# jdidion/atropos

Measured on AMD Instinct MI355X. Metric: reads/s (whole node) 150 bp SE adapter-align, higher is better.
Workload: dtype int32

## Files before the change

### atropos_amd/csrc/piece_kernels.hip

```cpp
#include "locate_fast.hpp"
#include "piece_filter.hpp"
#include "jit.hpp"

namespace atr {

void launch_fast_scan(FastWork wk, hipStream_t st);
int launch_fast_dp(const atr_aligner *a, const uint4 *packed, const int32_t *lens, long long nreads, int nchunks,
                   int max_len, uint4 *out, FastWork wk, const LinkedArgs *la, int idx, int count, hipStream_t st, bool planes, bool one_stream);

template <int NW, bool RAGGED, int WW>
__global__ __launch_bounds__(256) __attribute__((amdgpu_waves_per_eu(ATR_PIECE_WAVES(NW), 8))) void piece_filter_kernel(
    const LocateParams p, const FilterParams fp, const PieceParams pp, const uint4 *__restrict__ planes,
    const int32_t *__restrict__ lens, long long nreads, int max_len, uint4 *__restrict__ out, FastWork wk) {
    piece_filter_body<NW, RAGGED, WW>(p, fp, pp, planes, lens, nreads, max_len, out, wk);
}

__global__ __launch_bounds__(256) void piece_scatter_kernel(long long nreads, int m, FastWork wk) {
    __shared__ uint32_t s_cur[FILTER_BINS + 1], s_tmp[256];
    const long long ntiles = (nreads + 63) >> 6;
    long long t0, t1;
    block_tiles(ntiles, t0, t1, wk.nused);
    const uint2 *list = wk.tmp + t0 * 64;
    const uint32_t count = wk.lcount[blockIdx.x];
    const uint32_t mine = threadIdx.x < FILTER_BINS ? wk.counts[(size_t)blockIdx.x * FILTER_BINS + threadIdx.x] : 0u;
    const uint2 first = threadIdx.x < count ? list[threadIdx.x] : make_uint2(0u, 0u);
    if (wk.fused) {
        fused_bin_bases(wk, s_cur, s_tmp);
        if (threadIdx.x < FILTER_BINS) s_cur[threadIdx.x] += mine;
    } else if (threadIdx.x < FILTER_BINS) s_cur[threadIdx.x] = fast_slot0(wk, threadIdx.x);
    __syncthreads();
    for (uint32_t i = threadIdx.x; i < count; i += 256) {
        const uint2 e = i == threadIdx.x ? first : list[i];
        const uint32_t slot = atomicAdd(&s_cur[window_bin(e.y & ~PIECE_NODENSE, m, true)], 1u);
        wk.order[slot] = e;
        wk.dref[slot] = (uint32_t)(t0 * 64) + i;
    }
}

template <int NW, bool RAGGED, int WW>
static int piece_resident_blocks() {
    static thread_local int cached_dev = -1, cached = 0;
    int dev = 0;
    if (hipGetDevice(&dev) != hipSuccess) return 1024;
    if (dev != cached_dev) {
        int per_cu = 0, cus = 0;
        if (hipOccupancyMaxActiveBlocksPerMultiprocessor(&per_cu, piece_filter_kernel<NW, RAGGED, WW>, 256, 0) != hipSuccess || per_cu < 1) per_cu = 2;
        if (hipDeviceGetAttribute(&cus, hipDeviceAttributeMultiprocessorCount, dev) != hipSuccess || cus < 1) cus = 256;
        cached = std::min(FAST_BLOCKS, per_cu * cus);
        cached_dev = dev;
    }
    return cached;
}

template <int NW, int WW>
static void launch_piece_filter_w(const atr_aligner *a, const FilterParams &fp, const PieceParams &pp, const uint4 *planes,
                                  const int32_t *lens, long long nreads, int max_len, uint4 *out, FastWork &wk, hipStream_t st) {
    const long long want = ((nreads + 63) / 64 + 3) / 4;
    if (lens) {
        wk.nused = (int)std::max<long long>(1, std::min<long long>(piece_resident_blocks<NW, true, WW>(), want));
        hipLaunchKernelGGL((piece_filter_kernel<NW, true, WW>), dim3(wk.nused), dim3(256), 0, st, a->p, fp, pp, planes, lens, nreads, max_len, out, wk);
    } else {
        wk.nused = (int)std::max<long long>(1, std::min<long long>(piece_resident_blocks<NW, false, WW>(), want));
        hipLaunchKernelGGL((piece_filter_kernel<NW, false, WW>), dim3(wk.nused), dim3(256), 0, st, a->p, fp, pp, planes, lens, nreads, max_len, out, wk);
    }
}
template <int NW>
static void launch_piece_filter(const atr_aligner *a, const FilterParams &fp, const PieceParams &pp, const uint4 *planes,
                                const int32_t *lens, long long nreads, int max_len, uint4 *out, FastWork &wk, hipStream_t st) {
    if (pp.window > PIECE_WINDOW || pp.nb > 5 || fp.rows > 32) launch_piece_filter_w<NW, 3>(a, fp, pp, planes, lens, nreads, max_len, out, wk, st);
    else launch_piece_filter_w<NW, 2>(a, fp, pp, planes, lens, nreads, max_len, out, wk, st);
}

int piece_ragged_len(int max_len) { return 32 * ((max_len + 31) / 32); }
bool piece_applies(const atr_aligner *a, int max_len, FilterParams *fp_out, PieceParams *pp_out) {
    if (!a->filterable || max_len < 1) return false;
    const FilterParams &fp = aligner_piece_filter_params(a);
    PieceParams pp;
    if (!piece_params(a->codes, a->p.m, fp.rows, a->p.k, a->flags, a->wildcard_ref || a->wildcard_query,
                      a->table_kind == ATR_TABLE_CUSTOM, fp.thr_row, max_len, pp, a->p.thr, a->p.min_overlap, fp.cert, a->p.indel)) return false;
    const int nw = (max_len + 31) / 32;
    if (nw < 3 || nw > 10) return false;
    if (fp_out) *fp_out = fp;
    if (pp_out) *pp_out = pp;
    return true;
}

static const jit::SpecKernel *piece_spec_for(const atr_aligner *a, const FilterParams &fp, const PieceParams &pp, bool ragged,
                                             int max_len, long long nreads, bool force, int ascii_stride = 0) {
    const int pol = jit::policy();
    if (pol == 0) return nullptr;
    const int nw = (max_len + 31) / 32;
    a->planes_seen += nreads;
    const bool compile = force || pol == 1 || a->planes_seen >= jit::min_reads();
    return jit::spec_kernel(a, fp, pp, nw, ragged, ragged ? 32 * nw : max_len, compile, ascii_stride);
}

static bool tail_spec_enabled() {
    const char *x = getenv("ATR_TAIL_SPEC");
    return !(x && x[0] == '0');
}

int prepare_locate_planes(const atr_aligner *a, int max_len, bool ragged) {
    FilterParams fp;
    PieceParams pp;
    if (!piece_applies(a, ragged ? piece_ragged_len(max_len) : max_len, &fp, &pp)) return 0;
    return piece_spec_for(a, fp, pp, ragged, max_len, 0, true) != nullptr ? 1 : 0;
}

int launch_planes_prepass(const atr_aligner *a, const uint4 *planes, const int32_t *lens, long long nreads, int max_len,
                          uint4 *out, void *work, hipStream_t st, int grid_div, PlanesCall *pc) {
    FilterParams fp;
    PieceParams pp;
    if (!piece_applies(a, lens ? piece_ragged_len(max_len) : max_len, &fp, &pp)) return (int)hipErrorInvalidValue;
    FastWork wk = fast_carve(work, nreads);
    wk.lpw = nreads <= 8192 ? 0 : 64;
    const int nw = (max_len + 31) / 32;
    const jit::SpecKernel *sk = piece_spec_for(a, fp, pp, lens != nullptr, max_len, nreads, false);
    wk.fused = fast_fused_scan() ? 1 : 0;
    if (wk.fused) {
        const hipError_t rc = hipMemsetAsync(wk.chunks, 0, (size_t)wk.nbins * 4, st);
        if (rc != hipSuccess) return (int)rc;
    }
    if (sk) {
        const long long want = ((nreads + 63) / 64 + 3) / 4;
        wk.nused = (int)std::max<long long>(1, std::min<long long>(std::max(1, sk->resident / std::max(1, grid_div)), want));
        const hipError_t rc = jit::spec_launch(sk, wk.nused, planes, lens, nreads, max_len, out, wk, st);
        if (rc != hipSuccess) return (int)rc;
    } else {
        switch (nw) {
        case 3: launch_piece_filter<3>(a, fp, pp, planes, lens, nreads, max_len, out, wk, st); break;
        case 4: launch_piece_filter<4>(a, fp, pp, planes, lens, nreads, max_len, out, wk, st); break;
        case 5: launch_piece_filter<5>(a, fp, pp, planes, lens, nreads, max_len, out, wk, st); break;
        case 6: launch_piece_filter<6>(a, fp, pp, planes, lens, nreads, max_len, out, wk, st); break;
        case 7: launch_piece_filter<7>(a, fp, pp, planes, lens, nreads, max_len, out, wk, st); break;
        case 8: launch_piece_filter<8>(a, fp, pp, planes, lens, nreads, max_len, out, wk, st); break;
        case 9: launch_piece_filter<9>(a, fp, pp, planes, lens, nreads, max_len, out, wk, st); break;
        default: launch_piece_filter<10>(a, fp, pp, planes, lens, nreads, max_len, out, wk, st); break;
        }
    }
    pc->wk = wk;
    pc->nw = nw;
    pc->tail = sk ? (void *)sk->tail : nullptr;
    return (int)hipGetLastError();
}

int launch_planes_tail(const atr_aligner *a, const uint4 *planes, const int32_t *lens, long long nreads, int max_len, uint4 *out,
                       const PlanesCall &pc, hipStream_t st, bool one_stream) {
    FastWork wk = pc.wk;
    if (!wk.fused) launch_fast_scan(wk, st);
    hipLaunchKernelGGL(piece_scatter_kernel, dim3(wk.nused), dim3(256), 0, st, nreads, a->p.m, wk);
    if (pc.tail && !one_stream && tail_spec_enabled()) {
        {
            const bool small = nreads <= 65536;
            const int win_blocks = (int)std::max<long long>(1, std::min<long long>((nreads + 3) / 4, 1024));
            const int band_blocks = (int)std::max<long long>(1, std::min<long long>(small ? (nreads + 3) / 4 : (nreads + 255) / 256, 4096));
            const hipError_t rc = jit::tail_launch((hipFunction_t)pc.tail, win_blocks, band_blocks, planes, lens, pc.nw, max_len, out, wk, st);
            return rc != hipSuccess ? (int)rc : (int)hipGetLastError();
        }
    }
    return launch_fast_dp(a, planes, lens, nreads, pc.nw, max_len, out, wk, nullptr, 0, 1, st, true, one_stream);
}

int launch_locate_planes_shared(const atr_aligner *a, const uint4 *planes, const int32_t *lens, long long nreads, int max_len,
                                uint4 *out, void *work, hipStream_t st, int grid_div, bool one_stream) {
    PlanesCall pc;
    const int rc = launch_planes_prepass(a, planes, lens, nreads, max_len, out, work, st, grid_div, &pc);
    if (rc != 0) return rc;
    return launch_planes_tail(a, planes, lens, nreads, max_len, out, pc, st, one_stream);
}

int launch_locate_ascii_fused(const atr_aligner *a, const uint8_t *ascii, long long row_stride, const int32_t *lens, long long nreads,
                              int max_len, const uint8_t table[256], uint4 *planes, uint4 *out, void *work, hipStream_t st) {
    FilterParams fp;
    PieceParams pp;
    if (!piece_applies(a, lens ? piece_ragged_len(max_len) : max_len, &fp, &pp)) return 1;
    const int nw = (max_len + 31) / 32;
    static const bool off = [] { const char *x = getenv("ATR_ASCII_FUSED"); return x && x[0] == '0'; }();
    if (off || nw > 8 || row_stride < max_len || row_stride > 256 || ((uintptr_t)ascii & 1)) return 1;
    const jit::SpecKernel *sk = piece_spec_for(a, fp, pp, lens != nullptr, max_len, nreads, jit::policy() != 0, (int)row_stride);
    if (!sk) return 1;
    FastWork wk = fast_carve(work, nreads);
    wk.lpw = nreads <= 8192 ? 0 : 64;
    wk.fused = fast_fused_scan() ? 1 : 0;
    if (wk.fused) {
        const hipError_t rc = hipMemsetAsync(wk.chunks, 0, (size_t)wk.nbins * 4, st);
        if (rc != hipSuccess) return (int)rc;
    }
    const long long want = ((nreads + 63) / 64 + 3) / 4;
    wk.nused = (int)std::max<long long>(1, std::min<long long>(sk->resident, want));
    const hipError_t rc = jit::spec_launch_ascii(sk, wk.nused, ascii, lens, nreads, max_len, out, wk, planes, table, st);
    if (rc != hipSuccess) return (int)rc;
    PlanesCall pc;
    pc.wk = wk;
    pc.nw = nw;
    pc.tail = (void *)sk->tail;
    return launch_planes_tail(a, planes, lens, nreads, max_len, out, pc, st, false);
}

int launch_locate_planes(const atr_aligner *a, const uint4 *planes, const int32_t *lens, long long nreads, int max_len, uint4 *out,
                         void *work, hipStream_t st) {
    return launch_locate_planes_shared(a, planes, lens, nreads, max_len, out, work, st, 1, false);
}

}
```

### atropos_amd/csrc/tail_filter.hpp

```cpp
#ifndef ATR_TAIL_FILTER_HPP
#define ATR_TAIL_FILTER_HPP

#ifdef ATR_HOST_EMU
#include "filter_core.hpp"
#else
#include "fast_work.hpp"
#endif

namespace atr {

#ifndef ATR_TAIL_ROWS_UNROLL
#define ATR_TAIL_ROWS_UNROLL 8
#endif
#ifndef ATR_TAIL_WINDOW_UNROLL
#define ATR_TAIL_WINDOW_UNROLL 2
#endif
constexpr int TAIL_ROWS_UNROLL = ATR_TAIL_ROWS_UNROLL;
static_assert(TAIL_ROWS_UNROLL >= 8 && TAIL_ROWS_UNROLL % 8 == 0, "the feed position is a compile-time place of the body");

template <bool AND_MODE, int ND>
ATR_DEV void tail_band_row(const Uniform &u, uint32_t rrep, uint32_t qw0, uint32_t qw1, uint32_t (&band)[BAND_W]) {
    const uint32_t inf = ((uint32_t)INIT_COST_CAP << CSH) | ORG_BIAS;
    uint32_t m0 = nibble_any(AND_MODE ? (qw0 & rrep) : (qw0 ^ rrep));
    uint32_t m1 = ND > 8 ? nibble_any(AND_MODE ? (qw1 & rrep) : (qw1 ^ rrep)) : 0u;
    if (AND_MODE) { m0 = ~m0; m1 = ~m1; }
    uint32_t left = inf;
#pragma unroll
    for (int c = 0; c < ND; ++c) {
        const uint32_t bit = atr_bfe1(c < 8 ? m0 : m1, 4 * (c & 7) + 3);
        const uint32_t cd = atr_mad24(bit, COST1 + MATCH1, band[c]);
        const uint32_t up = c + 1 < ND ? band[c + 1 < ND ? c + 1 : 0] : inf;
        const uint32_t nw = atr_minu(atr_minu(cd, left + u.delw), up + u.insw) & ~PRIO_MASK;
        band[c] = nw;
        left = nw;
    }
}

struct TailLast {
    int cap_lo, top, r0, at0, n, cindel;
    bool active;
};

template <bool AND_MODE, int ND, int ROWS_MAX, bool LAST>
ATR_DEV void tail_band_sweep(const Uniform &u, const uint32_t *rreps, int rows, const uint32_t *ns, int nss,
                             uint32_t (&band)[BAND_W], const TailLast &tl, const int16_t *thr, Best &best) {
    uint32_t qw0 = ns[0], qw1 = ns[(size_t)nss];
    uint32_t feed = ns[(size_t)2 * nss];
#pragma unroll 1
    for (int i0 = 0; i0 < ROWS_MAX; i0 += TAIL_ROWS_UNROLL) {
        if (i0 >= rows) break;
#pragma unroll
        for (int t = 0; t < TAIL_ROWS_UNROLL; ++t) {
            const int i = i0 + t + 1;
            if (i <= ROWS_MAX && i <= rows) {
                tail_band_row<AND_MODE, ND>(u, rreps[i - 1], qw0, qw1, band);
                if (LAST && i >= tl.cap_lo) {
                    const int at = tl.at0 - i;
                    if (tl.active && i <= tl.top && i >= tl.r0 && (u.er || i == u.m)) {
                        uint32_t cell = band[0];
#pragma unroll
                        for (int c = 1; c < ND; ++c) cell = at == c ? band[c] : cell;
                        if (cell < u.klimit) consider<true>(best, cell, i, tl.n, u.min_overlap, thr, tl.cindel);
                    }
                }
                qw0 = (qw0 >> 4) | (qw1 << 28);
                qw1 = (qw1 >> 4) | (feed << 28);
                feed >>= 4;
                if (((t + 1) & 7) == 0) {
                    const int k = 2 + (i >> 3);
                    feed = k < BAND_STREAM ? ns[(size_t)k * nss] : 0u;
                }
            }
        }
    }
}

ATR_DEV void tail_band_record(const Best &best, int none_cost, uint32_t rec[4]) {
    const int cost = (int)(best.word >> CSH);
    int refstart = 0, querystart = 0, refstop = -1, querystop = 0, matches = 0, errors = 0;
    if (cost != none_cost) {
        const int origin = (int)(best.word & ORG_MASK) - (int)ORG_BIAS;
        if (origin >= 0) querystart = origin; else refstart = -origin;
        refstop = best.ref_stop; querystop = best.query_stop;
        matches = best.matches; errors = cost;
    }
    rec[0] = (uint32_t)(refstart & 0xFFFF) | ((uint32_t)(refstop & 0xFFFF) << 16);
    rec[1] = (uint32_t)(querystart & 0xFFFF) | ((uint32_t)(querystop & 0xFFFF) << 16);
    rec[2] = (uint32_t)(matches & 0xFFFF) | ((uint32_t)(errors & 0xFFFF) << 16);
    rec[3] = 0;
}

template <bool AND_MODE, int ROWS_MAX>
ATR_DEV void tail_band_locate(const Uniform &u, const uint32_t *rreps, bool noindel, const uint32_t *ns, int nss, int n,
                              uint32_t ww, int smax, const int16_t *thr, uint32_t rec[4]) {
    const int dlo = window_lo(ww);
    uint32_t band[BAND_W];
#pragma unroll
    for (int c = 0; c < BAND_W; ++c) band[c] = ORG_BIAS + (uint32_t)(dlo + c);
    Best best;
    best.key = COST_FIELD_MAX - (u.m + n);
    best.word = (uint32_t)(u.m + n) << CSH;
    best.ref_stop = u.m; best.query_stop = n; best.matches = 0;
    const TailLast none = {0, 0, 0, 0, 0, 0, false};
    if (smax < 8) tail_band_sweep<AND_MODE, 8, ROWS_MAX, false>(u, rreps, u.m, ns, nss, band, none, thr, best);
    else if (smax < 10) tail_band_sweep<AND_MODE, 10, ROWS_MAX, false>(u, rreps, u.m, ns, nss, band, none, thr, best);
    else if (smax < 12) tail_band_sweep<AND_MODE, 12, ROWS_MAX, false>(u, rreps, u.m, ns, nss, band, none, thr, best);
    else if (smax < 14) tail_band_sweep<AND_MODE, 14, ROWS_MAX, false>(u, rreps, u.m, ns, nss, band, none, thr, best);
    else tail_band_sweep<AND_MODE, 16, ROWS_MAX, false>(u, rreps, u.m, ns, nss, band, none, thr, best);
    const int cindel = noindel ? 0 : u.indel;
#pragma unroll
    for (int c = 0; c < BAND_W; ++c) {
        const int j = dlo + u.m + c;
        if (c <= smax && band[c] < u.klimit && j <= n) consider<true>(best, band[c], u.m, j, u.min_overlap, thr, cindel);
    }
    tail_band_record(best, u.m + n, rec);
}

template <bool AND_MODE, int ROWS_MAX>
ATR_DEV void tail_band_locate_last(const Uniform &u, const uint32_t *rreps, bool noindel, const uint32_t *ns, int nss, int n,
                                   uint32_t ww, bool active, int smax, int rows_max, int cap_lo, const int16_t *thr,
                                   uint32_t rec[4]) {
    const int dlo = window_lo(ww), top = window_rows(ww), r0 = top - last_band_span(ww), at0 = n - dlo;
    uint32_t band[BAND_W];
#pragma unroll
    for (int c = 0; c < BAND_W; ++c) band[c] = ORG_BIAS + (uint32_t)(dlo + c);
    Best best, bm;
    best.key = COST_FIELD_MAX - (u.m + n);
    best.word = (uint32_t)(u.m + n) << CSH;
    best.ref_stop = u.m; best.query_stop = n; best.matches = 0;
    bm = best;
    const int cindel = noindel ? 0 : u.indel;
    const TailLast tl = {cap_lo, top, r0, at0, n, cindel, active};
    if (smax < 4) tail_band_sweep<AND_MODE, 4, ROWS_MAX, true>(u, rreps, rows_max, ns, nss, band, tl, thr, best);
    else if (smax < 6) tail_band_sweep<AND_MODE, 6, ROWS_MAX, true>(u, rreps, rows_max, ns, nss, band, tl, thr, best);
    else if (smax < 8) tail_band_sweep<AND_MODE, 8, ROWS_MAX, true>(u, rreps, rows_max, ns, nss, band, tl, thr, best);
    else if (smax < 10) tail_band_sweep<AND_MODE, 10, ROWS_MAX, true>(u, rreps, rows_max, ns, nss, band, tl, thr, best);
    else if (smax < 12) tail_band_sweep<AND_MODE, 12, ROWS_MAX, true>(u, rreps, rows_max, ns, nss, band, tl, thr, best);
    else if (smax < 14) tail_band_sweep<AND_MODE, 14, ROWS_MAX, true>(u, rreps, rows_max, ns, nss, band, tl, thr, best);
    else tail_band_sweep<AND_MODE, 16, ROWS_MAX, true>(u, rreps, rows_max, ns, nss, band, tl, thr, best);
    if (last_band_rowm(ww) && rows_max == u.m) {
        const int width = last_band_width(ww);
#pragma unroll
        for (int c = 0; c < BAND_W; ++c) {
            const int j = dlo + u.m + c;
            if (c <= width && band[c] < u.klimit && j <= n) consider<true>(bm, band[c], u.m, j, u.min_overlap, thr, cindel);
        }
        if (bm.key >= best.key) best = bm;
    }
    tail_band_record(best, u.m + n, rec);
}

#if defined(ATR_TAIL_SPEC) && !defined(ATR_HOST_EMU)
#include "tail_spec_config.h"

__device__ __forceinline__ Uniform tail_uniform() {
    Uniform u;
    u.m = tspec::M; u.k = tspec::K; u.p0 = tspec::MT - tspec::M; u.indel = tspec::INDEL; u.min_overlap = tspec::MIN_OVERLAP;
    u.sr = (tspec::FLAGS & ATR_START_WITHIN_SEQ1) != 0; u.sq = (tspec::FLAGS & ATR_START_WITHIN_SEQ2) != 0;
    u.er = (tspec::FLAGS & ATR_STOP_WITHIN_SEQ1) != 0;  u.eq = (tspec::FLAGS & ATR_STOP_WITHIN_SEQ2) != 0;
    u.first_p = u.p0 + (u.er ? 0 : u.m);
    u.insw = (uint32_t)u.indel * COST1 + PRIO_INS;
    u.delw = (uint32_t)u.indel * COST1 + PRIO_DEL;
    u.klimit = (uint32_t)(u.k + 1) << CSH;
    return u;
}

__device__ __forceinline__ int tail_lanes_per_wave(long long tasks, long long grid_waves, int fixed) {
    if (fixed) return fixed;
    int lpw = 1;
    while (lpw < 64 && (long long)lpw * grid_waves < tasks) lpw <<= 1;
    return lpw;
}

struct TailShared {
    int16_t thr[tspec::M + 2];
    uint32_t init[tspec::MT + 1];
    __attribute__((aligned(16))) uint32_t nm[16][4];
    uint32_t stream[4][BAND_STREAM][64];
    uint32_t spread[4][256];
};

__device__ __forceinline__ void tail_band_blocks(TailShared &S, int block, int nblocks, const uint4 *__restrict__ packed,
                                                 const int32_t *__restrict__ lens, int nchunks, int max_len,
                                                 uint4 *__restrict__ out, const FastWork &wk) {
    constexpr int M = tspec::M;
    const Uniform u = tail_uniform();
    const long long total = (long long)wk.binbase[BAND_BINS];
    const int lane = threadIdx.x & 63, wave = __builtin_amdgcn_readfirstlane((int)(threadIdx.x >> 6));
    const long long stride = (long long)nblocks * 4;
    const int lpw = tail_lanes_per_wave(total, stride, wk.lpw);
    const long long nwaves = (total + lpw - 1) / lpw;
    uint32_t *ns = &S.stream[wave][0][lane];
    long long wv = (long long)block * 4 + wave;
    if (wv >= nwaves) return;
    auto slot_of = [&](long long w) { return w * lpw + lane; };
    auto live_of = [&](long long w) { return w < nwaves && lane < lpw && slot_of(w) < total; };
    auto dense_of = [&](long long w, uint2 task) { return live_of(w) && (task.y & PIECE_NODENSE) == 0u; };
    const uint4 zero4 = make_uint4(0u, 0u, 0u, 0u);
    uint2 task = live_of(wv) ? wk.order[slot_of(wv)] : make_uint2(0u, 0u);
    uint32_t di = live_of(wv) ? wk.dref[slot_of(wv)] : 0u;
    uint2 task1 = live_of(wv + stride) ? wk.order[slot_of(wv + stride)] : make_uint2(0u, 0u);
    uint32_t di1 = live_of(wv + stride) ? wk.dref[slot_of(wv + stride)] : 0u;
    uint4 a = dense_of(wv, task) ? wk.tdata[2 * (size_t)di] : zero4, b = dense_of(wv, task) ? wk.tdata[2 * (size_t)di + 1] : zero4;
    int n = live_of(wv) ? (lens ? lens[task.x] : max_len) : 0;
    for (; wv < nwaves; wv += stride) {
        const bool live = live_of(wv);
        const long long r = (long long)task.x;
        const uint32_t ww = task.y;
        const bool dense1 = dense_of(wv + stride, task1);
        const uint4 a1 = dense1 ? wk.tdata[2 * (size_t)di1] : zero4, b1 = dense1 ? wk.tdata[2 * (size_t)di1 + 1] : zero4;
        const int n1 = live_of(wv + stride) ? (lens ? lens[task1.x] : max_len) : 0;
        const bool live2 = live_of(wv + 2 * stride);
        const uint2 task2 = live2 ? wk.order[slot_of(wv + 2 * stride)] : make_uint2(0u, 0u);
        const uint32_t di2 = live2 ? wk.dref[slot_of(wv + 2 * stride)] : 0u;

        const bool last = live && window_scan(ww);
        const bool any_last = wave_max_i32(last ? 1 : 0) != 0, any_rowm = wave_max_i32(live && !last ? 1 : 0) != 0;
        const int s_lane = (live && !last) ? window_hi(ww) - u.m + u.k - window_lo(ww) : 0;
        const int smax = min(BAND_W - 1, wave_max_i32(s_lane));
        const bool dense = live && (ww & PIECE_NODENSE) == 0u;
        if (dense) {
            ns[0] = a.x; ns[64] = a.y; ns[128] = a.z; ns[192] = a.w;
            ns[256] = b.x; ns[320] = b.y; ns[384] = b.z; ns[448] = b.w;
        }
        if (wave_max_i32(live && !dense ? 1 : 0) != 0) {
            const uint32_t *q = (const uint32_t *)(packed + ((size_t)(r >> 6) * nchunks) * 64 + (r & 63));
            if (live && !dense) band_stage_planes(q, nchunks, window_lo(ww), ns, 64, S.spread, band_stream_dwords(M));
        }
        uint32_t rec[4] = {0xFFFF0000u, 0u, 0u, 0u};
        if (any_rowm) tail_band_locate<tspec::AND_MODE, M>(u, tspec::RREP, tspec::NOINDEL, ns, 64, n, ww, smax, S.thr, rec);
        if (any_last) {
            const int smax_l = min(BAND_W - 1, wave_max_i32(last ? last_band_width(ww) : 0));
            const int rows_max = wave_max_i32(last ? (last_band_rowm(ww) ? u.m : window_rows(ww)) : 0);
            const int cap_lo = wave_min_i32(last ? window_rows(ww) - last_band_span(ww) : 0x7fffffff);
            uint32_t rec_l[4];
            tail_band_locate_last<tspec::AND_MODE, M>(u, tspec::RREP, tspec::NOINDEL, ns, 64, n, ww, last, smax_l, min(rows_max, M), cap_lo, S.thr, rec_l);
            if (last) { rec[0] = rec_l[0]; rec[1] = rec_l[1]; rec[2] = rec_l[2]; rec[3] = rec_l[3]; }
        }
        if (live) out[r] = make_uint4(rec[0], rec[1], rec[2], rec[3]);
        task = task1; di = di1; a = a1; b = b1; n = n1;
        task1 = task2; di1 = di2;
    }
}

template <int W>
__device__ __forceinline__ void tail_load_mask(uint32_t (&nm)[W], const uint32_t (*s_nm)[4], uint32_t q) {
#pragma unroll
    for (int w = 0; w < W; ++w) nm[w] = s_nm[q][w];
}

__device__ __forceinline__ void tail_window_blocks(TailShared &S, int block, int nblocks, const uint4 *__restrict__ packed,
                                                   const int32_t *__restrict__ lens, int nchunks, int max_len,
                                                   uint4 *__restrict__ out, const FastWork &wk) {
    constexpr int MT = tspec::MT;
    constexpr bool NOINDEL = tspec::NOINDEL;
    const Uniform u = tail_uniform();
    const int16_t *s_thr = S.thr;
    const uint32_t *s_init = S.init;
    const uint32_t (*s_nm)[4] = S.nm;
    const uint32_t (*s_spread)[256] = S.spread;
    const long long first = (long long)wk.binbase[BAND_BINS], total = (long long)wk.binbase[FILTER_BINS];
    if (total <= first) return;
    const int lane = threadIdx.x & 63;
    const int lpw = tail_lanes_per_wave(total - first, (long long)nblocks * 4, wk.lpw);
    const long long nwaves = (total - first + lpw - 1) / lpw;
    __builtin_amdgcn_s_setprio(3);
    for (long long wv = (long long)block * 4 + __builtin_amdgcn_readfirstlane((int)(threadIdx.x >> 6)); wv < nwaves;
         wv += (long long)nblocks * 4) {
        const long long slot = first + wv * lpw + lane;
        const bool live = lane < lpw && slot < total;
        const uint2 task = live ? wk.order[slot] : make_uint2(0u, 0u);
        const long long r = (long long)task.x;
        const uint32_t ww = task.y;
        const int n = live ? (lens ? lens[r] : max_len) : 0;
        const int j_lo = window_lo(ww), j_hi = live ? window_hi(ww) : 0;
        const bool has_window = live && j_hi > j_lo;
        const int jlo = wave_min_i32(live ? j_lo : 0x7fffffff);
        const int jhi = wave_max_i32(has_window ? j_hi : 0);
        const int rows_w = wave_max_i32(live ? window_rows(ww) : 0);
        const int plimit = u.p0 + rows_w;
        const bool head = !(u.sr && jlo == 0);
        const bool rows_wave = __builtin_amdgcn_readfirstlane((int)(first + wv * lpw >= (long long)wk.binbase[ROWS_BIN0])) != 0;
        const bool tri = rows_wave && head && lens == nullptr;

        LaneState<MT> L;
        const uint4 *tp = packed + ((size_t)(r >> 6) * nchunks) * 64 + (r & 63);

        if (lens != nullptr && rows_wave && !u.sr) {
            const int shift = live ? max_len - n : 0;
            const int v0 = wave_min_i32(live ? j_lo + shift : 0x7fffffff);
            if (max_len - v0 <= TAIL_COLUMNS && v0 < max_len) {
                const int s_top_t = wave_max_i32(shift);
                lane_init_window<MT, NOINDEL>(L, u, max_len, v0, live ? max_len : 0, live && window_scan(ww), s_init, s_thr);
                uint32_t tb[TAIL_COLUMNS / 8];
                {
                    const int dlo = n - TAIL_COLUMNS;
                    const int z0 = dlo >> 3;
                    const uint32_t sh = 4u * (uint32_t)(dlo & 7);
                    uint32_t raw[TAIL_COLUMNS / 8 + 1];
#pragma unroll
                    for (int t = 0; t <= TAIL_COLUMNS / 8; ++t)
                        raw[t] = live ? read_dword_planes((const uint32_t *)tp, nchunks, z0 + t, s_spread) : 0u;
#pragma unroll
                    for (int t = 0; t < TAIL_COLUMNS / 8; ++t) tb[t] = sh ? ((raw[t] >> sh) | (raw[t + 1] << (32u - sh))) : raw[t];
                }
                int j = max_len - TAIL_COLUMNS;
#pragma unroll 1
                for (int d = 0; d < TAIL_COLUMNS / 8; ++d) {
                    uint32_t w = tb[0];
#pragma unroll
                    for (int t = 0; t + 1 < TAIL_COLUMNS / 8; ++t) tb[t] = tb[t + 1];
#pragma unroll 1
                    for (int b = 0; b < 8; ++b) {
                        ++j;
                        const uint32_t q = w & 15u;
                        w >>= 4;
                        if (j <= v0) continue;
                        uint32_t nm[(MT + 31) / 32];
                        tail_load_mask(nm, s_nm, q);
                        int pl = min(plimit, u.p0 + (j - v0) + u.k);
                        pl = min(pl, u.p0 + triangle_rows(rows_w, max_len, j, u.k));
                        lane_step<MT, NOINDEL, true, true>(L, u, j, nm, s_thr, pl);
                        if (j <= s_top_t && shift == j) lane_restart_window<MT>(L, u, j);
                    }
                }
                if (live) {
                    uint32_t rec[4];
                    lane_result<MT>(L, u, rec);
                    if ((rec[0] >> 16) != 0xFFFFu) rec[1] -= (uint32_t)shift * 0x00010001u;
                    out[r] = make_uint4(rec[0], rec[1], rec[2], rec[3]);
                }
                continue;
            }
        }
        lane_init_window<MT, NOINDEL>(L, u, n, jlo, j_hi, live && window_scan(ww), s_init, s_thr);
        if (jhi > jlo) {
            const int c0 = jlo >> 5, c1 = (jhi + 31) >> 5;
            uint4 nxt = tp[(size_t)c0 * 64];
            for (int c = c0; c < c1; ++c) {
                uint4 cur = nxt;
                if (c + 1 < c1) nxt = tp[(size_t)(c + 1) * 64];
                cur = make_uint4(piece_nibbles(s_spread, cur.x, cur.y, cur.z, cur.w, 0), piece_nibbles(s_spread, cur.x, cur.y, cur.z, cur.w, 1),
                                 piece_nibbles(s_spread, cur.x, cur.y, cur.z, cur.w, 2), piece_nibbles(s_spread, cur.x, cur.y, cur.z, cur.w, 3));
                int j = c * 32;
#pragma unroll 1
                for (int d = 0; d < 4; ++d) {
                    uint32_t w = cur.x;
                    cur.x = cur.y; cur.y = cur.z; cur.z = cur.w;
#pragma unroll ATR_TAIL_WINDOW_UNROLL
                    for (int b = 0; b < 8; ++b) {
                        ++j;
                        const uint32_t q = w & 15u;
                        w >>= 4;
                        if (j <= jlo || j > jhi) continue;
                        uint32_t nm[(MT + 31) / 32];
                        tail_load_mask(nm, s_nm, q);
                        int pl = head ? min(plimit, u.p0 + (j - jlo) + u.k) : plimit;
                        if (tri) pl = min(pl, u.p0 + triangle_rows(rows_w, max_len, j, u.k));
                        lane_step<MT, NOINDEL, true, true>(L, u, j, nm, s_thr, pl);
                    }
                }
            }
        }
        if (live) {
            uint32_t rec[4];
            lane_result<MT>(L, u, rec);
            out[r] = make_uint4(rec[0], rec[1], rec[2], rec[3]);
        }
    }
}

__device__ __forceinline__ void tail_body(const uint4 *__restrict__ packed, const int32_t *__restrict__ lens, int nchunks,
                                          int max_len, uint4 *__restrict__ out, const FastWork &wk, int win_blocks) {
    __shared__ TailShared S;
    for (int i = threadIdx.x; i <= tspec::MT + 1; i += 256) {
        if (i <= tspec::M + 1) S.thr[i] = tspec::THR[i];
        if (i <= tspec::MT) S.init[i] = init_word(i - (tspec::MT - tspec::M), 0, (tspec::FLAGS & ATR_START_WITHIN_SEQ1) != 0,
                                                  (tspec::FLAGS & ATR_START_WITHIN_SEQ2) != 0, tspec::INDEL);
    }
    if (threadIdx.x < 64) S.nm[threadIdx.x >> 2][threadIdx.x & 3] = tspec::NMASK[threadIdx.x >> 2][threadIdx.x & 3];
    piece_spread_fill(S.spread);
    __syncthreads();
    const int block = (int)blockIdx.x, nblocks = (int)gridDim.x;
    if (block < win_blocks) tail_window_blocks(S, block, win_blocks, packed, lens, nchunks, max_len, out, wk);
    else tail_band_blocks(S, block - win_blocks, nblocks - win_blocks, packed, lens, nchunks, max_len, out, wk);
}
#endif

}
#endif
```

Measured before the change: 24.46 billion.

## Split window-tail DP across four cooperating lanes per read using DPP

Adds a cooperative window path in which four lanes share one read's DP column. Each lane owns a quarter of the pattern positions and passes boundary cells to its neighbour with DPP quad shifts, skewed by one column per lane; best results are merged across the quad at the end. It is used when the number of window tasks is small, and is meant to cut per-lane register pressure and the serial work per lane, giving more parallelism. Blocks with no work now exit before filling shared memory, and an environment knob can cap the band block count. The cost is extra cross-lane shuffles, skew steps and more complex control flow.

```diff
diff --git a/atropos_amd/csrc/piece_kernels.hip b/atropos_amd/csrc/piece_kernels.hip
--- a/atropos_amd/csrc/piece_kernels.hip
+++ b/atropos_amd/csrc/piece_kernels.hip
@@ -99,6 +99,12 @@
     const char *x = getenv("ATR_TAIL_SPEC");
     return !(x && x[0] == '0');
 }
+static int tail_band_blocks_for(long long most) {
+    const char *x = getenv("ATR_TAIL_BAND_BLOCKS");
+    long long want = most;
+    if (x && *x) { const long long v = atoll(x); if (v >= 1) want = v; }
+    return (int)std::max<long long>(1, std::min(most, want));
+}
 
 int prepare_locate_planes(const atr_aligner *a, int max_len, bool ragged) {
     FilterParams fp;
@@ -153,7 +159,8 @@
         {
             const bool small = nreads <= 65536;
             const int win_blocks = (int)std::max<long long>(1, std::min<long long>((nreads + 3) / 4, 1024));
-            const int band_blocks = (int)std::max<long long>(1, std::min<long long>(small ? (nreads + 3) / 4 : (nreads + 255) / 256, 4096));
+            const long long most = std::max<long long>(1, std::min<long long>(small ? (nreads + 3) / 4 : (nreads + 255) / 256, 4096));
+            const int band_blocks = tail_band_blocks_for(most);
             const hipError_t rc = jit::tail_launch((hipFunction_t)pc.tail, win_blocks, band_blocks, planes, lens, pc.nw, max_len, out, wk, st);
             return rc != hipSuccess ? (int)rc : (int)hipGetLastError();
         }
diff --git a/atropos_amd/csrc/tail_filter.hpp b/atropos_amd/csrc/tail_filter.hpp
--- a/atropos_amd/csrc/tail_filter.hpp
+++ b/atropos_amd/csrc/tail_filter.hpp
@@ -150,6 +150,119 @@
     tail_band_record(best, u.m + n, rec);
 }
 
+#ifndef ATR_TAIL_WINDOW_LANES
+#define ATR_TAIL_WINDOW_LANES 4
+#endif
+static_assert(ATR_TAIL_WINDOW_LANES == 1 || ATR_TAIL_WINDOW_LANES == 4, "one lane per read, or four");
+#ifndef ATR_TAIL_COOP_MAX_TASKS
+#define ATR_TAIL_COOP_MAX_TASKS 32768
+#endif
+constexpr int COOP_LANES = 4, COOP_TASKS = 64 / COOP_LANES;
+
+struct CoopWave {
+    int jlo, jhi, plimit, rows_w, max_len;
+    bool head, tri;
+};
+
+template <int MT>
+struct CoopState {
+    uint32_t cell[MT / COOP_LANES];
+    uint32_t top;
+    Best bm, bl;
+    int n, max_n;
+    bool scan;
+};
+
+ATR_DEV uint32_t coop_mask_word(const uint32_t *nmask, int q, int R) {
+    const int lo = q * R, w = lo >> 5, s = lo & 31;
+    uint32_t v = nmask[w] >> s;
+    if (s != 0 && w + 1 < 4) v |= nmask[w + 1] << (32 - s);
+    return R < 32 ? v & ((1u << R) - 1u) : v;
+}
+
+ATR_DEV int coop_limit(const Uniform &u, const CoopWave &W, int j) {
+    int pl = W.head ? atr_min(W.plimit, u.p0 + (j - W.jlo) + u.k) : W.plimit;
+    if (W.tri) pl = atr_min(pl, u.p0 + triangle_rows(W.rows_w, W.max_len, j, u.k));
+    return pl;
+}
+
+template <int MT, bool NOINDEL>
+ATR_DEV void coop_scan(CoopState<MT> &C, const Uniform &u, int q, int last_p, const int16_t *thr) {
+    constexpr int R = MT / COOP_LANES;
+    const int indel = NOINDEL ? 0 : u.indel;
+    if (q == 0 && u.first_p <= 0 && last_p >= 0 && C.top < u.klimit) consider<true>(C.bl, C.top, -u.p0, C.n, u.min_overlap, thr, indel);
+#pragma unroll
+    for (int r = 0; r < R; ++r) {
+        const int pos = q * R + 1 + r;
+        if (pos >= u.first_p && pos <= last_p && C.cell[r] < u.klimit) consider<true>(C.bl, C.cell[r], pos - u.p0, C.n, u.min_overlap, thr, indel);
+    }
+}
+
+template <int MT, bool NOINDEL>
+ATR_DEV void coop_init(CoopState<MT> &C, const Uniform &u, int q, int n, int j_start, int j_hi, bool scan, const uint32_t *s_init,
+                       const int16_t *thr) {
+    constexpr int R = MT / COOP_LANES;
+    static_assert(MT % COOP_LANES == 0 && R <= 32, "a quarter of the positions, one mask word");
+    C.n = n; C.max_n = j_hi; C.scan = scan;
+    C.top = j_start == 0 ? s_init[q * R] : window_init_word(q * R - u.p0, j_start, u.indel);
+#pragma unroll
+    for (int r = 0; r < R; ++r) C.cell[r] = j_start == 0 ? s_init[q * R + 1 + r] : window_init_word(q * R + 1 + r - u.p0, j_start, u.indel);
+    C.bm.key = COST_FIELD_MAX - (u.m + n);
+    C.bm.word = (uint32_t)(u.m + n) << CSH;
+    C.bm.ref_stop = u.m; C.bm.query_stop = n; C.bm.matches = 0;
+    C.bl = C.bm;
+    if (scan && j_hi <= j_start) coop_scan<MT, NOINDEL>(C, u, q, MT, thr);
+}
+
+template <int MT, bool NOINDEL, class X>
+ATR_DEV void coop_step(CoopState<MT> &C, const Uniform &u, const CoopWave &W, int q, int j, uint32_t nmw, const int16_t *thr, const X &x) {
+    constexpr int R = MT / COOP_LANES;
+    const uint32_t recv = x.up(C.cell[R - 1]);
+    if (j <= W.jlo || j > W.jhi) return;
+    const uint32_t row0 = u.sq ? (ORG_BIAS + (uint32_t)j) : (ORG_BIAS | ((uint32_t)atr_min(j * u.indel, INIT_COST_CAP) << CSH));
+    const uint32_t top_new = q == 0 ? row0 : recv;
+    uint32_t cd = atr_mad24(atr_bfe1(nmw, 0), COST1 + MATCH1, C.top);
+    uint32_t up = top_new;
+#pragma unroll
+    for (int r = 0; r < R; ++r) {
+        uint32_t cd_next = 0;
+        if (r + 1 < R) cd_next = atr_mad24(atr_bfe1(nmw, r + 1), COST1 + MATCH1, C.cell[r]);
+        uint32_t nw;
+        if (NOINDEL) {
+            nw = cd;
+        } else {
+            const uint32_t cl = C.cell[r] + u.delw;
+            const uint32_t cu = up + u.insw;
+            nw = atr_minu(atr_minu(cd, cl), cu) & ~PRIO_MASK;
+        }
+        if (r + 1 < ROW_GRAN) nw = (q * R + r + 1 == u.p0) ? row0 : nw;
+        C.cell[r] = nw;
+        up = nw;
+        cd = cd_next;
+    }
+    C.top = top_new;
+    if (q == COOP_LANES - 1) {
+        const uint32_t wm = C.cell[R - 1];
+        if (wm < u.klimit && j <= C.max_n && coop_limit(u, W, j) == MT)
+            consider<true>(C.bm, wm, u.m, j, u.min_overlap, thr, NOINDEL ? 0 : u.indel);
+    }
+    if (C.scan && j == C.max_n && C.max_n > W.jlo) coop_scan<MT, NOINDEL>(C, u, q, coop_limit(u, W, j), thr);
+}
+
+template <int MT, class X>
+ATR_DEV bool coop_finish(const CoopState<MT> &C, const Uniform &u, int q, uint32_t rec[4], const X &x) {
+    LaneState<MT> L;
+    L.best = C.bm;
+    const Best b0 = x.template best_of<0>(C.bl), b1 = x.template best_of<1>(C.bl), b2 = x.template best_of<2>(C.bl);
+    if (b0.key > L.best.key) L.best = b0;
+    if (b1.key > L.best.key) L.best = b1;
+    if (b2.key > L.best.key) L.best = b2;
+    if (C.bl.key > L.best.key) L.best = C.bl;
+    L.n = C.n;
+    lane_result<MT>(L, u, rec);
+    return q == COOP_LANES - 1;
+}
+
 #if defined(ATR_TAIL_SPEC) && !defined(ATR_HOST_EMU)
 #include "tail_spec_config.h"
 
@@ -176,6 +289,7 @@
     int16_t thr[tspec::M + 2];
     uint32_t init[tspec::MT + 1];
     __attribute__((aligned(16))) uint32_t nm[16][4];
+    __attribute__((aligned(16))) uint32_t nmq[16][COOP_LANES];
     uint32_t stream[4][BAND_STREAM][64];
     uint32_t spread[4][256];
 };
@@ -249,9 +363,9 @@
     for (int w = 0; w < W; ++w) nm[w] = s_nm[q][w];
 }
 
-__device__ __forceinline__ void tail_window_blocks(TailShared &S, int block, int nblocks, const uint4 *__restrict__ packed,
-                                                   const int32_t *__restrict__ lens, int nchunks, int max_len,
-                                                   uint4 *__restrict__ out, const FastWork &wk) {
+__device__ __forceinline__ void tail_window_wave(TailShared &S, long long base, int lpw, long long total, const uint4 *__restrict__ packed,
+                                                 const int32_t *__restrict__ lens, int nchunks, int max_len,
+                                                 uint4 *__restrict__ out, const FastWork &wk) {
     constexpr int MT = tspec::MT;
     constexpr bool NOINDEL = tspec::NOINDEL;
     const Uniform u = tail_uniform();
@@ -259,129 +373,242 @@
     const uint32_t *s_init = S.init;
     const uint32_t (*s_nm)[4] = S.nm;
     const uint32_t (*s_spread)[256] = S.spread;
-    const long long first = (long long)wk.binbase[BAND_BINS], total = (long long)wk.binbase[FILTER_BINS];
-    if (total <= first) return;
     const int lane = threadIdx.x & 63;
-    const int lpw = tail_lanes_per_wave(total - first, (long long)nblocks * 4, wk.lpw);
-    const long long nwaves = (total - first + lpw - 1) / lpw;
-    __builtin_amdgcn_s_setprio(3);
-    for (long long wv = (long long)block * 4 + __builtin_amdgcn_readfirstlane((int)(threadIdx.x >> 6)); wv < nwaves;
-         wv += (long long)nblocks * 4) {
-        const long long slot = first + wv * lpw + lane;
-        const bool live = lane < lpw && slot < total;
-        const uint2 task = live ? wk.order[slot] : make_uint2(0u, 0u);
-        const long long r = (long long)task.x;
-        const uint32_t ww = task.y;
-        const int n = live ? (lens ? lens[r] : max_len) : 0;
-        const int j_lo = window_lo(ww), j_hi = live ? window_hi(ww) : 0;
-        const bool has_window = live && j_hi > j_lo;
-        const int jlo = wave_min_i32(live ? j_lo : 0x7fffffff);
-        const int jhi = wave_max_i32(has_window ? j_hi : 0);
-        const int rows_w = wave_max_i32(live ? window_rows(ww) : 0);
-        const int plimit = u.p0 + rows_w;
-        const bool head = !(u.sr && jlo == 0);
-        const bool rows_wave = __builtin_amdgcn_readfirstlane((int)(first + wv * lpw >= (long long)wk.binbase[ROWS_BIN0])) != 0;
-        const bool tri = rows_wave && head && lens == nullptr;
-
-        LaneState<MT> L;
-        const uint4 *tp = packed + ((size_t)(r >> 6) * nchunks) * 64 + (r & 63);
-
-        if (lens != nullptr && rows_wave && !u.sr) {
-            const int shift = live ? max_len - n : 0;
-            const int v0 = wave_min_i32(live ? j_lo + shift : 0x7fffffff);
-            if (max_len - v0 <= TAIL_COLUMNS && v0 < max_len) {
-                const int s_top_t = wave_max_i32(shift);
-                lane_init_window<MT, NOINDEL>(L, u, max_len, v0, live ? max_len : 0, live && window_scan(ww), s_init, s_thr);
-                uint32_t tb[TAIL_COLUMNS / 8];
-                {
-                    const int dlo = n - TAIL_COLUMNS;
-                    const int z0 = dlo >> 3;
-                    const uint32_t sh = 4u * (uint32_t)(dlo & 7);
-                    uint32_t raw[TAIL_COLUMNS / 8 + 1];
-#pragma unroll
-                    for (int t = 0; t <= TAIL_COLUMNS / 8; ++t)
-                        raw[t] = live ? read_dword_planes((const uint32_t *)tp, nchunks, z0 + t, s_spread) : 0u;
-#pragma unroll
-                    for (int t = 0; t < TAIL_COLUMNS / 8; ++t) tb[t] = sh ? ((raw[t] >> sh) | (raw[t + 1] << (32u - sh))) : raw[t];
-                }
-                int j = max_len - TAIL_COLUMNS;
+    const long long slot = base + lane;
+    const bool live = lane < lpw && slot < total;
+    const uint2 task = live ? wk.order[slot] : make_uint2(0u, 0u);
+    const long long r = (long long)task.x;
+    const uint32_t ww = task.y;
+    const int n = live ? (lens ? lens[r] : max_len) : 0;
+    const int j_lo = window_lo(ww), j_hi = live ? window_hi(ww) : 0;
+    const bool has_window = live && j_hi > j_lo;
+    const int jlo = wave_min_i32(live ? j_lo : 0x7fffffff);
+    const int jhi = wave_max_i32(has_window ? j_hi : 0);
+    const int rows_w = wave_max_i32(live ? window_rows(ww) : 0);
+    const int plimit = u.p0 + rows_w;
+    const bool head = !(u.sr && jlo == 0);
+    const bool rows_wave = __builtin_amdgcn_readfirstlane((int)(base >= (long long)wk.binbase[ROWS_BIN0])) != 0;
+    const bool tri = rows_wave && head && lens == nullptr;
+
+    LaneState<MT> L;
+    const uint4 *tp = packed + ((size_t)(r >> 6) * nchunks) * 64 + (r & 63);
+
+    if (lens != nullptr && rows_wave && !u.sr) {
+        const int shift = live ? max_len - n : 0;
+        const int v0 = wave_min_i32(live ? j_lo + shift : 0x7fffffff);
+        if (max_len - v0 <= TAIL_COLUMNS && v0 < max_len) {
+            const int s_top_t = wave_max_i32(shift);
+            lane_init_window<MT, NOINDEL>(L, u, max_len, v0, live ? max_len : 0, live && window_scan(ww), s_init, s_thr);
+            uint32_t tb[TAIL_COLUMNS / 8];
+            {
+                const int dlo = n - TAIL_COLUMNS;
+                const int z0 = dlo >> 3;
+                const uint32_t sh = 4u * (uint32_t)(dlo & 7);
+                uint32_t raw[TAIL_COLUMNS / 8 + 1];
+#pragma unroll
+                for (int t = 0; t <= TAIL_COLUMNS / 8; ++t)
+                    raw[t] = live ? read_dword_planes((const uint32_t *)tp, nchunks, z0 + t, s_spread) : 0u;
+#pragma unroll
+                for (int t = 0; t < TAIL_COLUMNS / 8; ++t) tb[t] = sh ? ((raw[t] >> sh) | (raw[t + 1] << (32u - sh))) : raw[t];
+            }
+            int j = max_len - TAIL_COLUMNS;
 #pragma unroll 1
-                for (int d = 0; d < TAIL_COLUMNS / 8; ++d) {
-                    uint32_t w = tb[0];
-#pragma unroll
-                    for (int t = 0; t + 1 < TAIL_COLUMNS / 8; ++t) tb[t] = tb[t + 1];
+            for (int d = 0; d < TAIL_COLUMNS / 8; ++d) {
+                uint32_t w = tb[0];
+#pragma unroll
+                for (int t = 0; t + 1 < TAIL_COLUMNS / 8; ++t) tb[t] = tb[t + 1];
 #pragma unroll 1
-                    for (int b = 0; b < 8; ++b) {
-                        ++j;
-                        const uint32_t q = w & 15u;
-                        w >>= 4;
-                        if (j <= v0) continue;
-                        uint32_t nm[(MT + 31) / 32];
-                        tail_load_mask(nm, s_nm, q);
-                        int pl = min(plimit, u.p0 + (j - v0) + u.k);
-                        pl = min(pl, u.p0 + triangle_rows(rows_w, max_len, j, u.k));
-                        lane_step<MT, NOINDEL, true, true>(L, u, j, nm, s_thr, pl);
-                        if (j <= s_top_t && shift == j) lane_restart_window<MT>(L, u, j);
-                    }
-                }
-                if (live) {
-                    uint32_t rec[4];
-                    lane_result<MT>(L, u, rec);
-                    if ((rec[0] >> 16) != 0xFFFFu) rec[1] -= (uint32_t)shift * 0x00010001u;
-                    out[r] = make_uint4(rec[0], rec[1], rec[2], rec[3]);
-                }
-                continue;
-            }
-        }
-        lane_init_window<MT, NOINDEL>(L, u, n, jlo, j_hi, live && window_scan(ww), s_init, s_thr);
-        if (jhi > jlo) {
-            const int c0 = jlo >> 5, c1 = (jhi + 31) >> 5;
-            uint4 nxt = tp[(size_t)c0 * 64];
-            for (int c = c0; c < c1; ++c) {
-                uint4 cur = nxt;
-                if (c + 1 < c1) nxt = tp[(size_t)(c + 1) * 64];
-                cur = make_uint4(piece_nibbles(s_spread, cur.x, cur.y, cur.z, cur.w, 0), piece_nibbles(s_spread, cur.x, cur.y, cur.z, cur.w, 1),
-                                 piece_nibbles(s_spread, cur.x, cur.y, cur.z, cur.w, 2), piece_nibbles(s_spread, cur.x, cur.y, cur.z, cur.w, 3));
-                int j = c * 32;
-#pragma unroll 1
-                for (int d = 0; d < 4; ++d) {
-                    uint32_t w = cur.x;
-                    cur.x = cur.y; cur.y = cur.z; cur.z = cur.w;
-#pragma unroll ATR_TAIL_WINDOW_UNROLL
-                    for (int b = 0; b < 8; ++b) {
-                        ++j;
-                        const uint32_t q = w & 15u;
-                        w >>= 4;
-                        if (j <= jlo || j > jhi) continue;
-                        uint32_t nm[(MT + 31) / 32];
-                        tail_load_mask(nm, s_nm, q);
-                        int pl = head ? min(plimit, u.p0 + (j - jlo) + u.k) : plimit;
-                        if (tri) pl = min(pl, u.p0 + triangle_rows(rows_w, max_len, j, u.k));
-                        lane_step<MT, NOINDEL, true, true>(L, u, j, nm, s_thr, pl);
-                    }
+                for (int b = 0; b < 8; ++b) {
+                    ++j;
+                    const uint32_t q = w & 15u;
+                    w >>= 4;
+                    if (j <= v0) continue;
+                    uint32_t nm[(MT + 31) / 32];
+                    tail_load_mask(nm, s_nm, q);
+                    int pl = min(plimit, u.p0 + (j - v0) + u.k);
+                    pl = min(pl, u.p0 + triangle_rows(rows_w, max_len, j, u.k));
+                    lane_step<MT, NOINDEL, true, true>(L, u, j, nm, s_thr, pl);
+                    if (j <= s_top_t && shift == j) lane_restart_window<MT>(L, u, j);
                 }
             }
-        }
-        if (live) {
-            uint32_t rec[4];
-            lane_result<MT>(L, u, rec);
-            out[r] = make_uint4(rec[0], rec[1], rec[2], rec[3]);
-        }
+            if (live) {
+                uint32_t rec[4];
+                lane_result<MT>(L, u, rec);
+                if ((rec[0] >> 16) != 0xFFFFu) rec[1] -= (uint32_t)shift * 0x00010001u;
+                out[r] = make_uint4(rec[0], rec[1], rec[2], rec[3]);
+            }
+            return;
+        }
+    }
+    lane_init_window<MT, NOINDEL>(L, u, n, jlo, j_hi, live && window_scan(ww), s_init, s_thr);
+    if (jhi > jlo) {
+        const int c0 = jlo >> 5, c1 = (jhi + 31) >> 5;
+        uint4 nxt = tp[(size_t)c0 * 64];
+        for (int c = c0; c < c1; ++c) {
+            uint4 cur = nxt;
+            if (c + 1 < c1) nxt = tp[(size_t)(c + 1) * 64];
+            cur = make_uint4(piece_nibbles(s_spread, cur.x, cur.y, cur.z, cur.w, 0), piece_nibbles(s_spread, cur.x, cur.y, cur.z, cur.w, 1),
+                             piece_nibbles(s_spread, cur.x, cur.y, cur.z, cur.w, 2), piece_nibbles(s_spread, cur.x, cur.y, cur.z, cur.w, 3));
+            int j = c * 32;
+#pragma unroll 1
+            for (int d = 0; d < 4; ++d) {
+                uint32_t w = cur.x;
+                cur.x = cur.y; cur.y = cur.z; cur.z = cur.w;
+#pragma unroll ATR_TAIL_WINDOW_UNROLL
+                for (int b = 0; b < 8; ++b) {
+                    ++j;
+                    const uint32_t q = w & 15u;
+                    w >>= 4;
+                    if (j <= jlo || j > jhi) continue;
+                    uint32_t nm[(MT + 31) / 32];
+                    tail_load_mask(nm, s_nm, q);
+                    int pl = head ? min(plimit, u.p0 + (j - jlo) + u.k) : plimit;
+                    if (tri) pl = min(pl, u.p0 + triangle_rows(rows_w, max_len, j, u.k));
+                    lane_step<MT, NOINDEL, true, true>(L, u, j, nm, s_thr, pl);
+                }
+            }
+        }
+    }
+    if (live) {
+        uint32_t rec[4];
+        lane_result<MT>(L, u, rec);
+        out[r] = make_uint4(rec[0], rec[1], rec[2], rec[3]);
+    }
+}
+
+struct QuadDpp {
+    __device__ __forceinline__ uint32_t up(uint32_t v) const {
+        return (uint32_t)__builtin_amdgcn_update_dpp((int)v, (int)v, 0x90, 0xF, 0xF, false);
+    }
+    template <int S>
+    __device__ __forceinline__ Best best_of(const Best &b) const {
+        Best r;
+        r.key = __builtin_amdgcn_update_dpp(b.key, b.key, S * 0x55, 0xF, 0xF, false);
+        r.word = (uint32_t)__builtin_amdgcn_update_dpp((int)b.word, (int)b.word, S * 0x55, 0xF, 0xF, false);
+        r.ref_stop = __builtin_amdgcn_update_dpp(b.ref_stop, b.ref_stop, S * 0x55, 0xF, 0xF, false);
+        r.query_stop = __builtin_amdgcn_update_dpp(b.query_stop, b.query_stop, S * 0x55, 0xF, 0xF, false);
+        r.matches = __builtin_amdgcn_update_dpp(b.matches, b.matches, S * 0x55, 0xF, 0xF, false);
+        return r;
+    }
+};
+
+__device__ __forceinline__ void tail_window_wave_coop(TailShared &S, long long base, int tpw, long long total, const uint4 *__restrict__ packed,
+                                                      const int32_t *__restrict__ lens, int nchunks, int max_len,
+                                                      uint4 *__restrict__ out, const FastWork &wk) {
+    constexpr int MT = tspec::MT;
+    constexpr bool NOINDEL = tspec::NOINDEL;
+    const Uniform u = tail_uniform();
+    const int lane = threadIdx.x & 63, q = lane & (COOP_LANES - 1), g = lane / COOP_LANES;
+    const long long slot = base + g;
+    const bool live = g < tpw && slot < total;
+    const uint2 task = live ? wk.order[slot] : make_uint2(0u, 0u);
+    const long long r = (long long)task.x;
+    const uint32_t ww = task.y;
+    const int n = live ? (lens ? lens[r] : max_len) : 0;
+    const int j_lo = window_lo(ww), j_hi = live ? window_hi(ww) : 0;
+    const bool has_window = live && j_hi > j_lo;
+    const int jlo = wave_min_i32(live ? j_lo : 0x7fffffff);
+    const int jhi = wave_max_i32(has_window ? j_hi : 0);
+    const int rows_w = wave_max_i32(live ? window_rows(ww) : 0);
+    const bool head = !(u.sr && jlo == 0);
+    const bool rows_wave = __builtin_amdgcn_readfirstlane((int)(base >= (long long)wk.binbase[ROWS_BIN0])) != 0;
+    const CoopWave W = {jlo, jhi, u.p0 + rows_w, rows_w, max_len, head, rows_wave && head && lens == nullptr};
+    const QuadDpp x;
+    CoopState<MT> C;
+    coop_init<MT, NOINDEL>(C, u, q, n, jlo, j_hi, live && window_scan(ww), S.init, S.thr);
+    if (jhi > jlo) {
+        const uint4 *tp = packed + ((size_t)(r >> 6) * nchunks) * 64 + (r & 63);
+        const int c0 = jlo >> 5, c1 = (jhi + 31) >> 5, jend = jhi + COOP_LANES - 1;
+        const uint32_t sh = 4u * (uint32_t)q;
+        uint32_t hist = 0u, mask = 0u;
+        int jw = c0 * 32;
+        auto advance = [&](uint32_t code) {
+            ++jw;
+            hist = (hist << 4) | code;
+            const uint32_t next = S.nmq[(hist >> sh) & 15u][q];
+            if (jw - 1 > jlo && jw - 1 <= jend) coop_step<MT, NOINDEL>(C, u, W, q, jw - 1 - q, mask, S.thr, x);
+            mask = next;
+        };
+        uint4 nxt = tp[(size_t)c0 * 64];
+        for (int c = c0; c < c1; ++c) {
+            uint4 cur = nxt;
+            if (c + 1 < c1) nxt = tp[(size_t)(c + 1) * 64];
+            cur = make_uint4(piece_nibbles(S.spread, cur.x, cur.y, cur.z, cur.w, 0), piece_nibbles(S.spread, cur.x, cur.y, cur.z, cur.w, 1),
+                             piece_nibbles(S.spread, cur.x, cur.y, cur.z, cur.w, 2), piece_nibbles(S.spread, cur.x, cur.y, cur.z, cur.w, 3));
+#pragma unroll 1
+            for (int d = 0; d < 4; ++d) {
+                uint32_t w = cur.x;
+                cur.x = cur.y; cur.y = cur.z; cur.z = cur.w;
+#pragma unroll ATR_TAIL_WINDOW_UNROLL
+                for (int b = 0; b < 8; ++b) {
+                    advance(w & 15u);
+                    w >>= 4;
+                }
+            }
+        }
+#pragma unroll 1
+        while (jw <= jend) advance(0u);
+    }
+    uint32_t rec[4];
+    const bool mine = coop_finish<MT>(C, u, q, rec, x);
+    if (live && mine) out[r] = make_uint4(rec[0], rec[1], rec[2], rec[3]);
+}
+
+struct WindowWaves {
+    long long first, split, total, na, nb;
+    int tpw, lpw;
+};
+__device__ __forceinline__ WindowWaves tail_window_waves(const FastWork &wk, const int32_t *lens, int nblocks) {
+    WindowWaves v;
+    v.first = (long long)wk.binbase[BAND_BINS];
+    v.total = (long long)wk.binbase[FILTER_BINS];
+    v.split = v.first;
+    if (ATR_TAIL_WINDOW_LANES == COOP_LANES && v.total - v.first <= (long long)ATR_TAIL_COOP_MAX_TASKS) {
+        const bool tail_mode = lens != nullptr && (tspec::FLAGS & ATR_START_WITHIN_SEQ1) == 0;
+        v.split = tail_mode ? max(v.first, min(v.total, (long long)wk.binbase[ROWS_BIN0])) : v.total;
+    }
+    v.tpw = min(COOP_TASKS, tail_lanes_per_wave(v.split - v.first, (long long)nblocks * 4, wk.lpw));
+    v.lpw = tail_lanes_per_wave(v.total - v.split, (long long)nblocks * 4, wk.lpw);
+    v.na = (v.split - v.first + v.tpw - 1) / v.tpw;
+    v.nb = (v.total - v.split + v.lpw - 1) / v.lpw;
+    return v;
+}
+
+__device__ __forceinline__ void tail_window_blocks(TailShared &S, int block, int nblocks, const uint4 *__restrict__ packed,
+                                                   const int32_t *__restrict__ lens, int nchunks, int max_len,
+                                                   uint4 *__restrict__ out, const FastWork &wk) {
+    const WindowWaves v = tail_window_waves(wk, lens, nblocks);
+    __builtin_amdgcn_s_setprio(3);
+    for (long long wv = (long long)block * 4 + __builtin_amdgcn_readfirstlane((int)(threadIdx.x >> 6)); wv < v.na + v.nb;
+         wv += (long long)nblocks * 4) {
+        if (wv < v.na) tail_window_wave_coop(S, v.first + wv * v.tpw, v.tpw, v.split, packed, lens, nchunks, max_len, out, wk);
+        else tail_window_wave(S, v.split + (wv - v.na) * v.lpw, v.lpw, v.total, packed, lens, nchunks, max_len, out, wk);
     }
 }
 
 __device__ __forceinline__ void tail_body(const uint4 *__restrict__ packed, const int32_t *__restrict__ lens, int nchunks,
                                           int max_len, uint4 *__restrict__ out, const FastWork &wk, int win_blocks) {
     __shared__ TailShared S;
+    const int block = (int)blockIdx.x, nblocks = (int)gridDim.x;
+    if (block < win_blocks) {
+        const WindowWaves v = tail_window_waves(wk, lens, win_blocks);
+        if ((long long)block * 4 >= v.na + v.nb) return;
+    } else {
+        const long long total = (long long)wk.binbase[BAND_BINS], stride = (long long)(nblocks - win_blocks) * 4;
+        const int lpw = tail_lanes_per_wave(total, stride, wk.lpw);
+        if ((long long)(block - win_blocks) * 4 >= (total + lpw - 1) / lpw) return;
+    }
     for (int i = threadIdx.x; i <= tspec::MT + 1; i += 256) {
         if (i <= tspec::M + 1) S.thr[i] = tspec::THR[i];
         if (i <= tspec::MT) S.init[i] = init_word(i - (tspec::MT - tspec::M), 0, (tspec::FLAGS & ATR_START_WITHIN_SEQ1) != 0,
                                                   (tspec::FLAGS & ATR_START_WITHIN_SEQ2) != 0, tspec::INDEL);
     }
-    if (threadIdx.x < 64) S.nm[threadIdx.x >> 2][threadIdx.x & 3] = tspec::NMASK[threadIdx.x >> 2][threadIdx.x & 3];
+    if (threadIdx.x < 64) {
+        S.nm[threadIdx.x >> 2][threadIdx.x & 3] = tspec::NMASK[threadIdx.x >> 2][threadIdx.x & 3];
+        S.nmq[threadIdx.x >> 2][threadIdx.x & 3] = coop_mask_word(tspec::NMASK[threadIdx.x >> 2], (int)(threadIdx.x & 3), tspec::MT / COOP_LANES);
+    }
     piece_spread_fill(S.spread);
     __syncthreads();
-    const int block = (int)blockIdx.x, nblocks = (int)gridDim.x;
     if (block < win_blocks) tail_window_blocks(S, block, win_blocks, packed, lens, nchunks, max_len, out, wk);
     else tail_band_blocks(S, block - win_blocks, nblocks - win_blocks, packed, lens, nchunks, max_len, out, wk);
 }
```

After: 24.13 billion. -1.4%, worse.
